# nkwangyh/CubemapSLAM

Measured on AMD Instinct MI355X. Metric: frames/sec (extract+match+localBA) on Lafida cam0, higher is better.
Workload: dtype u8 (extract/match), f64 (BA)

## Files before the change

cubemapslam_amd/api.py:

```python
import time
import ctypes as C
import os
import numpy as np

_HERE = os.path.dirname(os.path.abspath(__file__))
LIB_PATH = os.environ.get("CMS_HIP_LIB") or os.path.join(_HERE, "lib", "libcubemapslam_hip.so")


class CmsError(RuntimeError):
    pass


class Camera(C.Structure):
    _fields_ = [("c", C.c_double), ("d", C.c_double), ("e", C.c_double), ("u0", C.c_double), ("v0", C.c_double),
                ("invpol", C.c_double * 12), ("pol", C.c_double * 5), ("Iw", C.c_int), ("Ih", C.c_int),
                ("face", C.c_int), ("fov_deg", C.c_double)]


class OrbParams(C.Structure):
    _fields_ = [("nfeatures", C.c_int), ("scale_factor", C.c_float), ("nlevels", C.c_int),
                ("ini_th_fast", C.c_int), ("min_th_fast", C.c_int)]


class Geometry(C.Structure):
# ... 795 lines not shown
        return lib().cms_ba_stream(self.h)

    def set_stream(self, hip_stream):
        f = lib().cms_ba_set_stream
        f.argtypes = [C.c_void_p, C.c_void_p]
        _chk(f(self.h, C.c_void_p(int(hip_stream))), "cms_ba_set_stream")

    def profile_kernel(self, kernel_id):
        _chk(lib().cms_ba_profile_kernel(self.h, kernel_id), "cms_ba_profile_kernel")

    def profile_get(self):
        ms = C.c_double(0); n = C.c_long(0)
        _chk(lib().cms_ba_profile_get(self.h, C.byref(ms), C.byref(n)), "cms_ba_profile_get")
        return ms.value, n.value

    def close(self):
        if getattr(self, "h", None) and self.h.value:
            lib().cms_ba_destroy(self.h)
            self.h = C.c_void_p()

    def __del__(self):
        try:
            self.close()
        except Exception:
            pass


def ba_compose_chunks(fixed, n_points, e_pose, e_point, lookahead=48):
    fixed = np.ascontiguousarray(fixed, np.uint8); e_pose = np.ascontiguousarray(e_pose, np.int32); e_point = np.ascontiguousarray(e_point, np.int32)
    P, E = int(n_points), len(e_pose)
# ... 89 lines not shown
    pp = (C.c_void_p * n)(*[o[0].ctypes.data for o in outs]); pq = (C.c_void_p * n)(*[o[1].ctypes.data for o in outs]); pf = (C.c_void_p * n)(*[o[2].ctypes.data for o in outs])
    L = lib()
    L.cms_ba_read_many.argtypes = [C.c_void_p, C.c_int, C.c_void_p, C.c_void_p, C.c_void_p]
    _chk(L.cms_ba_read_many(handles, n, pp, pq, pf), "cms_ba_read_many")
    return outs


def ba_pool_trim(device=0):
    n = C.c_size_t(0)
    L = lib()
    L.cms_ba_pool_trim.argtypes = [C.c_int, C.c_void_p]
    _chk(L.cms_ba_pool_trim(int(device), C.byref(n)), "cms_ba_pool_trim")
    return int(n.value)


def ba_set_deterministic(on):
    _chk(lib().cms_ba_set_deterministic(int(on) if not isinstance(on, bool) else (1 if on else 0)), "cms_ba_set_deterministic")


def ba_get_deterministic():
    return bool(lib().cms_ba_get_deterministic())


def ba_optimize_many(bas, its=(5, 10), stop=None, stop_array=None):
    n = len(bas)
    handles = (C.c_void_p * n)(*[b.h for b in bas])
    stats = (BaStats * n)()
    stop_arr = stop_array if stop_array is not None else (np.array([1], np.uint8) if stop else None)
    lib().cms_ba_optimize_many.argtypes = [C.c_void_p, C.c_int, C.c_int, C.c_int, C.c_void_p, C.c_void_p]
    rc = _chk(lib().cms_ba_optimize_many(handles, n, its[0], its[1], _p(stop_arr), stats), "cms_ba_optimize_many")
# ... 205 lines not shown
```

cubemapslam_amd/csrc/cms_api_ba.hip:

```cpp
#include <algorithm>
#include <cfloat>
#include <chrono>
#include <condition_variable>
#include <deque>
#include <functional>
#include <atomic>
#include <cmath>
#include <mutex>
#include <numeric>
#include <string>
#include <thread>
#include <pthread.h>
#include <unordered_map>
#include "cms_ba_pool.h"

struct BaKnobs {
  bool deterministic, det_points, host_lm, single_host_lm, schur_chunks, schur_points, all_lists, want_all_lists;
  bool no_fused, solve1, trial_points, fixed_ranges, no_permute, create_timing, compose_timing, runs, runs_as_edges, separate_reduce, separate_reduce2, separate_first_pass, rm_valu;
  int solve_reduce_max, leftover_lookahead;
  bool global_sum;
  int lookahead, compose_segments, dup, run_min_chunks, rm_weight, se_waves_cap, em_cost_a, em_cost_b, te_chunks, run_min_pct; bool unified;
  char stream_priority;
  bool run_wg; int rw_waves_cu0, rw_waves_cu1;
};
static const BaKnobs& ba_knobs() {
  static const BaKnobs k = [] {
    BaKnobs q;
    auto on = [](const char* n) { return getenv(n) != nullptr; };
    auto num = [](const char* n, int dflt) { const char* v = getenv(n); return v ? atoi(v) : dflt; };
    q.deterministic = on("CMS_BA_DETERMINISTIC"); q.host_lm = on("CMS_BA_HOST_LM"); q.single_host_lm = on("CMS_BA_SINGLE_HOST_LM");
    q.schur_chunks = on("CMS_BA_SCHUR_CHUNKS"); q.schur_points = on("CMS_BA_SCHUR_POINTS"); q.all_lists = on("CMS_BA_ALL_LISTS");
    q.det_points = on("CMS_BA_DET_POINTS");
    q.want_all_lists = (q.deterministic && q.det_points) || q.host_lm || q.single_host_lm || q.schur_chunks || q.schur_points || q.all_lists;
    q.no_fused = on("CMS_BA_NO_FUSED_LIN"); q.solve1 = on("CMS_BA_SOLVE1"); q.trial_points = on("CMS_BA_TRIAL_POINTS");
    q.fixed_ranges = on("CMS_BA_FIXED_RANGES"); q.no_permute = on("CMS_BA_NO_PERMUTE");
    q.create_timing = on("CMS_BA_CREATE_TIMING"); q.compose_timing = on("CMS_BA_COMPOSE_TIMING");
    q.runs = !on("CMS_BA_NO_RUNS");
    q.runs_as_edges = on("CMS_BA_RUNS_AS_EDGES");
// ... 2 lines not shown
    q.separate_reduce2 = on("CMS_BA_SEPARATE_REDUCE2");
    q.separate_reduce = on("CMS_BA_SEPARATE_REDUCE");
    { const char* v = getenv("CMS_BA_SOLVE_REDUCE_MAX"); q.solve_reduce_max = v ? atoi(v) : 24; }
    q.global_sum = !on("CMS_BA_NO_GLOBAL_SUM");
    q.leftover_lookahead = num("CMS_BA_LEFTOVER_LOOKAHEAD", 0);
    q.lookahead = num("CMS_BA_LOOKAHEAD", 24); q.compose_segments = num("CMS_BA_COMPOSE_SEGMENTS", 0); q.dup = num("CMS_BA_DUP", 0);
    q.run_min_chunks = std::max(1, num("CMS_BA_RUN_MIN_CHUNKS", q.rm_valu ? 2 : 1));
    q.run_min_pct = std::max(10, std::min(100, num("CMS_BA_RUN_MIN_PCT", 100)));
    q.rm_weight = std::max(10, std::min(400, num("CMS_BA_RM_WEIGHT", 58)));
    q.unified = !on("CMS_BA_SPLIT_WORKGROUPS");
    q.em_cost_a = num("CMS_BA_EM_COST_A", 40); q.em_cost_b = num("CMS_BA_EM_COST_B", 30);
    q.te_chunks = std::max(1, std::min(16, num("CMS_BA_TE_CHUNKS", 2)));
    q.se_waves_cap = num("CMS_BA_SE_WAVES", 0);
    q.run_wg = on("CMS_BA_RUN_WG");
    q.rw_waves_cu0 = std::max(1, std::min(32, num("CMS_BA_RW_WAVES0", 12))); q.rw_waves_cu1 = std::max(1, std::min(32, num("CMS_BA_RW_WAVES1", 8)));
    const char* pr = getenv("CMS_BA_STREAM_PRIORITY");
    q.stream_priority = pr ? pr[0] : 0;
    return q;
  }();
  return k;
}

struct BaExpand;
struct BaDevPlan;
struct BaCreateOpts {
  hipStream_t setup_stream = nullptr;
  bool inputs_pinned = false;
  bool force_host_plan = false;
  BaDevPlan* dev_plan = nullptr;
  BaExpand* defer_expand = nullptr;
// ... 25 lines not shown
  int* d_sp_pair_slots = nullptr; double* d_sp_partial = nullptr; double* d_sp_sum = nullptr; int* d_sp_chunk_off = nullptr;
  int sp_threads = 0; size_t sp_lds = 0;
  BaSe se = {};
  int* d_se_chunk_e0 = nullptr; uint32_t* d_se_info = nullptr; double* d_se_partial = nullptr; double* d_se_bp_partial = nullptr; double* d_se_sum = nullptr; int* d_se_pob = nullptr; int* d_se_chunk_off = nullptr;
  int* d_se_lone = nullptr; int4* d_rm_chunk = nullptr; uint2* d_run_lane = nullptr; uint32_t* d_run_mf = nullptr; uint32_t* d_run_fl = nullptr; uint32_t* d_rm_cost = nullptr;
  uint32_t* d_run_fg = nullptr; int* d_rm_cut = nullptr;
  size_t se_lds_fixed = 0; int se_waves = 0;
  size_t rm_lds = 0; int n_runs = 0, rm_points = 0;
  char* h_stage = nullptr; size_t h_stage_bytes = 0;
  int cur = 0;
  double* h_pin = nullptr; size_t h_pin_bytes = 0;
  void* grp_items_dev = nullptr; void* grp_items_host = nullptr; double* grp_scal_dev = nullptr; double* grp_scal_host = nullptr;
  void* grp_lm_dev = nullptr; void* grp_lm_host = nullptr;
  int grp_cap = 0;
  int prof_kernel = 0; std::vector<hipEvent_t> prof_ev; double prof_ms = 0; long prof_launches = 0;
  bool fast_plan = false;
  int* d_raw_pose = nullptr; int* d_raw_point = nullptr; int8_t* d_raw_face = nullptr; int* d_prank = nullptr; int* d_cpo = nullptr; int* d_cedge = nullptr;
  uint8_t* d_pcopy = nullptr; uint8_t* d_lo_copy = nullptr; uint64_t* d_run_sig = nullptr; int* d_iperm = nullptr;
  bool dev_plan = false;
  int* d_plan_counts = nullptr; int* h_plan_counts = nullptr; size_t h_plan_counts_bytes = 0;
  long long* d_plan_clk = nullptr;
  bool se_only = false;
  bool deterministic = false;
  int det_ranges = 0;
  bool det_points = false;
  hipEvent_t ev_setup = nullptr;
  bool setup_wait_pending = false;
  hipStream_t grp_stream = nullptr;
  bool async_pending = false;
  bool gsum_clean = false;
// ... 1615 lines not shown
```

cubemapslam_amd/csrc/cms_api_ba_lm.hip:

```cpp

struct BaLm {
  int iterations = 0, robust = 0;
  double delta = 0;
  int it = 0, qmax = 0, nBad = 0, done = 0, next = 0;
  double lambda = -1, ni = 2, currentChi = 0, iniChi = 0, rho = 0;
  double chi_ini = 0, chi_fin = 0, lam_fin = 0;
};

static bool ba_stopped(const volatile uint8_t* stop) { return stop && *stop; }

static int ba_enqueue_iter_start(cms_ba* b, const BaLm& st) {
  hipStream_t s = b->stream;
  const int cur = b->cur;
  ba_errors(b, cur, st.robust, st.delta, 0);
  hipLaunchKernelGGL(k_ba_lin_points, dim3(b->nblk_p), dim3(128), 0, s, b->d, (const double*)b->d_poses[cur],
                     (const double*)b->d_pts[cur], st.robust, st.delta, b->d_Hll, b->d_bl, b->d_Hpl);
  hipLaunchKernelGGL(k_ba_lin_poses, dim3(b->K, BA_POSE_CHUNKS), dim3(256), 0, s, b->d, (const double*)b->d_poses[cur],
                     (const double*)b->d_pts[cur], st.robust, st.delta, b->d_pose_partial);
  if (b->np > 0)
    hipLaunchKernelGGL(k_ba_pose_finish, dim3(b->np), dim3(64), 0, s, b->np, (const double*)b->d_pose_partial, b->d_Hpp, b->d_bp);
  if (st.it == 0) {
    HIPCHK(hipMemsetAsync(b->d_scal + 3, 0, sizeof(double), s));
    hipLaunchKernelGGL(k_ba_maxdiag, dim3(64), dim3(256), 0, s, b->np, b->P, (const double*)b->d_Hpp, (const double*)b->d_Hll, b->d_scal + 3);
  }
// ... 121 lines not shown
  return true;
}
static int ba_group_reserve(cms_ba* owner, int n) {
  if (owner->grp_cap >= n) return CMS_OK;
  if (owner->grp_items_host) ba_pin_give(owner->device, owner->grp_items_host, owner->grp_pin_bytes[0]);
  if (owner->grp_scal_host) ba_pin_give(owner->device, owner->grp_scal_host, owner->grp_pin_bytes[1]);
  if (owner->grp_lm_host) ba_pin_give(owner->device, owner->grp_lm_host, owner->grp_pin_bytes[2]);
  owner->grp_items_host = nullptr; owner->grp_scal_host = nullptr; owner->grp_lm_host = nullptr;
  owner->grp_cap = 0;
  const int cap = std::max(n, 8);
  { char* q = nullptr; int rc = ba_alloc(owner, &q, (size_t)cap * sizeof(BaItem)); if (rc) return rc; owner->grp_items_dev = q; }
  { int rc = ba_alloc(owner, &owner->grp_scal_dev, (size_t)cap * 8); if (rc) return rc; }
  { char* q = nullptr; int rc = ba_alloc(owner, &q, (size_t)cap * sizeof(BaLmDev)); if (rc) return rc; owner->grp_lm_dev = q; }
  HIPCHK(ba_pin_take(owner->device, (size_t)cap * sizeof(BaItem), &owner->grp_items_host, &owner->grp_pin_bytes[0]));
  HIPCHK(ba_pin_take(owner->device, (size_t)cap * 8 * sizeof(double), (void**)&owner->grp_scal_host, &owner->grp_pin_bytes[1]));
  HIPCHK(ba_pin_take(owner->device, (size_t)cap * sizeof(BaLmDev), &owner->grp_lm_host, &owner->grp_pin_bytes[2]));
  n = cap;
  owner->grp_cap = n;
  return CMS_OK;
}
static bool ba_all_sp(cms_ba** bas, int n) {
  for (int w = 0; w < n; ++w) if (bas[w]->sp.R <= 0) return false;
  return true;
}
static bool ba_use_se(cms_ba** bas, int n) {
  if (ba_knobs().host_lm) return false;
  for (int w = 0; w < n; ++w) if (bas[w]->se.nchunks <= 0 || bas[w]->det_points) return false;
  return true;
}
static bool ba_use_te(cms_ba** bas, int n) {
  if (ba_knobs().trial_points || !ba_use_se(bas, n)) return false;
// ... 147 lines not shown
      hipLaunchKernelGGL(kb_ba_trial_solve, dim3(1, 1, n), dim3(384), lds, s, ditems, dyn, (int)BA_PHASE_TRIAL);
      hipLaunchKernelGGL(kb_ba_trial_points, dim3(max_p, 1, n), dim3(128), 0, s, ditems, dyn, (int)BA_PHASE_TRIAL);
      hipLaunchKernelGGL(kb_ba_reduce2, dim3(1, 1, n), dim3(256), 0, s, ditems, dyn, (int)BA_PHASE_TRIAL);
    }
    HIPCHK(hipStreamSynchronize(s));
    for (int w = 0; w < n; ++w) {
      if (dyn.phase[w] == BA_PHASE_IDLE) continue;
      memcpy(bas[w]->h_pin, g->grp_scal_host + 8 * w, 8 * sizeof(double));
      if (dyn.phase[w] == BA_PHASE_ITER) ba_finish_iter_start(bas[w], st[w]);
      else ba_finish_trial(bas[w], st[w], stop);
    }
  }
  HIPCHK(hipGetLastError());
  return CMS_OK;
}
static int ba_optimize_stage_batched_dev(cms_ba** bas, int n, std::vector<BaLm>& st, const volatile uint8_t* stop) {
  cms_ba* g = bas[0];
  hipStream_t s = g->stream;
  const BaItem* ditems = reinterpret_cast<const BaItem*>(g->grp_items_dev);
  int max_e = 0, max_p = 0, max_K = 0, max_np = 0, max_chunks = 0, max_P = 0, max_R = 0, max_spt = 64, max_pairs = 0, max_it = 0;
  size_t lds = 0, sp_lds = 0;
  const bool all_sp = ba_all_sp(bas, n);
  for (int w = 0; w < n; ++w) {
    max_R = std::max(max_R, bas[w]->sp.R); max_spt = std::max(max_spt, bas[w]->sp_threads); max_pairs = std::max(max_pairs, bas[w]->npairs);
    sp_lds = std::max(sp_lds, bas[w]->sp_lds);
    max_e = std::max(max_e, bas[w]->nblk_e); max_p = std::max(max_p, bas[w]->nblk_p); max_K = std::max(max_K, bas[w]->K);
    max_np = std::max(max_np, bas[w]->np); max_chunks = std::max(max_chunks, bas[w]->nchunks); max_P = std::max(max_P, bas[w]->P);
    lds = std::max(lds, bas[w]->blk_lds);
    max_it = std::max(max_it, st[w].iterations);
  }
  BaLmDev* hlm = reinterpret_cast<BaLmDev*>(g->grp_lm_host);
  for (int w = 0; w < n; ++w) {
    BaLmDev& L = hlm[w];
    memset(&L, 0, sizeof(L));
    L.lambda = st[w].lambda; L.ni = st[w].ni; L.it = st[w].it; L.iterations = st[w].iterations; L.nBad = st[w].nBad; L.done = st[w].done;
    L.cur = bas[w]->cur;
    L.next = (st[w].it >= st[w].iterations || ba_stopped(stop)) ? 2 : 0;
  }
  hipLaunchKernelGGL(kb_ba_lm_load, dim3((n + 63) / 64), dim3(64), 0, s, ditems, n, st[0].robust ? 1 : 0);
  BaDyn dyn{};
  memset(&dyn, 0, sizeof(dyn));
  dyn.robust = st[0].robust; dyn.delta = st[0].delta; dyn.chi2_th = 5.991; dyn.set_level = 0; dyn.dev_lm = 1; dyn.fold_finish = 1;
  bool first_round = false;
  for (int w = 0; w < n; ++w) first_round = first_round || st[w].it == 0;
  const BaGroupMode gm = ba_group_mode(bas, n);
  const bool use_se = gm.use_se, use_te = gm.use_te;
  bool iter_phase = true;
  const bool use_s3 = gm.use_s3;
  int s3_threads = 64; size_t lds3 = 0;
  for (int w = 0; w < n; ++w) { s3_threads = std::max(s3_threads, ba_s3_threads(bas[w]->np)); lds3 = std::max(lds3, bas[w]->blk3_lds); }
  {
    static const int solve_kb = [] { const char* v = getenv("CMS_BA_SOLVE_LDS_KB"); return v ? atoi(v) : 0; }();
    if (solve_kb > 0) lds3 = std::max(lds3, std::min((size_t)solve_kb * 1024, (size_t)BA_LDS_CEILING));
  }
// ... 17 lines not shown
  const bool fused = gm.fused;
  const bool solve_reduces = fused && (gm.gsum || (!ba_knobs().separate_reduce && max_seR <= ba_knobs().solve_reduce_max));
  dyn.fused_lin = fused ? 1 : 0;
  {
    static const bool no_presum = getenv("CMS_BA_NO_SOLVE_PRESUM") != nullptr;
    const size_t need = lds3 + (size_t)max_np2 * 42 * sizeof(double);
    if (use_s3 && solve_reduces && !gm.gsum && !no_presum && need <= BA_LDS_CEILING) { dyn.solve_presum = 1; lds3 = need; }
  }
  const bool first_pass = fused && use_te && first_round && !ba_knobs().separate_first_pass;
  dyn.fold_reduce = (use_te && !ba_knobs().separate_reduce2 && ba_knobs().dup == 0) ? 1 : 0;
  int k = 0;
  const int pk = g->prof_kernel;
  const int dup = ba_knobs().dup;
  auto bracket = [&](int id, int which) {
    if (pk != id) return;
    const size_t i = 2 * (size_t)k + which;
    while (g->prof_ev.size() <= i) { hipEvent_t e = nullptr; if (hipEventCreate(&e) != hipSuccess) return; g->prof_ev.push_back(e); }
    hipEventRecord(g->prof_ev[i], s);
  };
  auto enqueue_round = [&]() {
      if (first_round && first_pass) {
        bracket(1, 0);
        hipLaunchKernelGGL(kb_ba_first_pass, dim3(max_Rt, 1, n), dim3(BA_TE_THREADS), te_lds, s, ditems, dyn, (int)BA_PHASE_ITER);
        bracket(1, 1);
        iter_phase = false;
      } else if (first_round) {
        hipLaunchKernelGGL(kb_ba_errors, dim3(max_e, 1, n), dim3(256), 0, s, ditems, dyn, (int)BA_PHASE_ITER);
        hipLaunchKernelGGL(kb_ba_reduce, dim3(1, 1, n), dim3(256), 0, s, ditems, dyn, (int)BA_PHASE_ITER);
      }
      first_round = false;
      if (iter_phase) {
// ... 65 lines not shown
      if (use_te) {
        hipLaunchKernelGGL(kb_ba_trial_edges, dim3(max_Rt, 1, n), dim3(BA_TE_THREADS), te_lds, s, ditems, dyn, (int)BA_PHASE_TRIAL);
        if (dup == 6) hipLaunchKernelGGL(kb_ba_trial_edges, dim3(max_Rt, 1, n), dim3(BA_TE_THREADS), te_lds, s, ditems, dyn, (int)BA_PHASE_TRIAL);
      } else {
        hipLaunchKernelGGL(kb_ba_trial_points, dim3(max_p, 1, n), dim3(128), 0, s, ditems, dyn, (int)BA_PHASE_TRIAL);
        if (dup == 6) hipLaunchKernelGGL(kb_ba_trial_points, dim3(max_p, 1, n), dim3(128), 0, s, ditems, dyn, (int)BA_PHASE_TRIAL);
      }
      bracket(6, 1);
      bracket(7, 0);
      if (!dyn.fold_reduce) hipLaunchKernelGGL(kb_ba_reduce2, dim3(1, 1, n), dim3(256), 0, s, ditems, dyn, (int)BA_PHASE_TRIAL);
      bracket(7, 1);
      ++k;
  };
  const volatile BaLmDev* vh = reinterpret_cast<const volatile BaLmDev*>(hlm);
  hipError_t werr = hipSuccess;
  for (long spins = 0;;) {
    bool any = false;
    for (int w = 0; w < n; ++w) any = any || vh[w].next != 2;
    if (!any || (k > 0 && ba_stopped(stop))) break;
    if (k - vh[0].rounds < (stop ? 1 : 2)) { enqueue_round(); spins = 0; continue; }
    if (spins < 256) std::this_thread::yield();
    else std::this_thread::sleep_for(std::chrono::microseconds(20));
    if ((++spins & 0xFFF) == 0 && hipStreamQuery(s) != hipErrorNotReady) {
      werr = hipStreamSynchronize(s);
      if (werr != hipSuccess || k - vh[0].rounds >= 2) { if (werr == hipSuccess) werr = hipErrorUnknown; break; }
    }
  }
  const hipError_t serr = hipStreamSynchronize(s);
  HIPCHK(werr);
  HIPCHK(serr);
  HIPCHK(hipGetLastError());
  if (pk > 0)
    for (int r = 0; r < k && 2 * (size_t)r + 1 < g->prof_ev.size(); ++r) {
      float ms = 0;
      if (hipEventElapsedTime(&ms, g->prof_ev[2 * r], g->prof_ev[2 * r + 1]) == hipSuccess) { g->prof_ms += ms; ++g->prof_launches; }
    }
  for (int w = 0; w < n; ++w) {
    const BaLmDev& L = hlm[w];
    BaLm& t = st[w];
    t.lambda = L.lambda; t.ni = L.ni; t.currentChi = L.currentChi; t.iniChi = L.iniChi; t.rho = L.rho; t.it = L.it; t.qmax = L.qmax;
    t.nBad = L.nBad; t.done = L.done; t.next = 2;
    if (L.done > 0 || L.it > 0) { t.chi_ini = L.chi_ini; t.chi_fin = L.chi_fin; t.lam_fin = L.lam_fin; }
    if (L.next == 1 && L.qmax > 0 && ba_stopped(stop)) {
      ++t.done; t.chi_ini = L.chi_ini; t.chi_fin = L.currentChi; t.lam_fin = L.lambda;
    }
    bas[w]->cur = L.cur;
  }
  return CMS_OK;
}

static int ba_classify_batched(cms_ba** bas, int n, int set_level, std::vector<int>& counts) {
  cms_ba* g = bas[0];
  hipStream_t s = g->stream;
  BaDyn dyn{};
  memset(&dyn, 0, sizeof(dyn));
  dyn.chi2_th = 5.991; dyn.set_level = set_level;
  int max_e = 0;
  for (int w = 0; w < n; ++w) {
    dyn.phase[w] = BA_PHASE_CLASSIFY; dyn.cur[w] = (uint8_t)bas[w]->cur;
    max_e = std::max(max_e, bas[w]->nblk_e);
  }
  const BaItem* ditems = reinterpret_cast<const BaItem*>(g->grp_items_dev);
  hipLaunchKernelGGL(kb_ba_classify, dim3(max_e, 1, n), dim3(256), 0, s, ditems, dyn, (int)BA_PHASE_CLASSIFY);
  hipLaunchKernelGGL(kb_ba_counts_publish, dim3((n + 63) / 64), dim3(64), 0, s, ditems, n);
  HIPCHK(hipStreamSynchronize(s));
  const BaLmDev* hlm = reinterpret_cast<const BaLmDev*>(g->grp_lm_host);
  counts.resize(n);
  for (int w = 0; w < n; ++w) counts[w] = hlm[w].n_out[set_level ? 0 : 1];
  return CMS_OK;
}

static int ba_optimize_group(cms_ba** bas, int n, int its_robust, int its_final, const volatile uint8_t* stop, cms_ba_stats* stats);
extern "C" int cms_ba_optimize_many(cms_ba** bas, int n, int its_robust, int its_final, const volatile uint8_t* stop, cms_ba_stats* stats) {
  if (!bas || n < 1) return cms_fail(CMS_ERR_ARG, "cms_ba_optimize_many: bad argument");
  for (int w = 0; w < n; ++w) if (!bas[w]) return cms_fail(CMS_ERR_ARG, "null ba");
  auto kind = [&](int w) {
    const cms_ba* b = bas[w];
    int k = b->device * 8 + (b->fast_plan ? 4 : 0) + (b->se.nchunks > 0 ? 2 : 0) + (b->deterministic ? 1 : 0);
    if (b->deterministic) k += 1024 * (1 + (b->det_points ? 1 : 0) + 2 * (b->rm_lds > 0 ? 1 : 0) + 4 * std::max(0, std::min(15, b->se_waves)) + 64 * b->det_ranges);
    return k;
// ... 47 lines not shown
  }
  std::vector<cms_ba_stats> local(n);
  for (int w = 0; w < n; ++w) memset(&local[w], 0, sizeof(cms_ba_stats));
  if (ba_stopped(stop)) {
    if (batched) for (int w = 0; w < n; ++w) bas[w]->gsum_clean = bas[w]->grp_se.gsum != 0;
    if (stats) memcpy(stats, local.data(), n * sizeof(cms_ba_stats));
    return 1;
  }
  const double delta = std::sqrt(5.991);
  std::vector<BaLm> st(n);
  for (int w = 0; w < n; ++w) { st[w] = BaLm(); st[w].iterations = its_robust; st[w].robust = 1; st[w].delta = delta; }
  const bool host_lm = ba_knobs().host_lm;
  for (int w = 0; w < n; ++w)
    if (bas[w]->se_only && (!batched || host_lm || !ba_use_se(bas, n)))
      return cms_fail(CMS_ERR_UNSUPPORTED, "cms_ba_optimize: the window carries only the edge-major work list but another kernel path was selected");
  int rc = batched ? (host_lm ? ba_optimize_stage_batched(bas, n, st, stop) : ba_optimize_stage_batched_dev(bas, n, st, stop)) : ba_optimize_stage_many(bas, n, st, stop);
  if (rc) return rc;
  tick("stage1");
  for (int w = 0; w < n; ++w) {
    local[w].iterations_done[0] = st[w].done; local[w].chi2_initial[0] = st[w].chi_ini; local[w].chi2_final[0] = st[w].chi_fin;
    local[w].lambda_final[0] = st[w].lam_fin;
  }
  std::vector<std::vector<uint8_t>> flags(n);
  std::vector<int> counts(n, 0);
  auto classify = [&](int set_level) -> int {
    if (batched) return ba_classify_batched(bas, n, set_level, counts);
    for (int w = 0; w < n; ++w) {
      cms_ba* b = bas[w];
      HIPCHK(hipSetDevice(b->device));
      flags[w].resize(b->E);
      hipLaunchKernelGGL(k_ba_classify, dim3(b->nblk_e), dim3(256), 0, b->stream, b->d, (const double*)b->d_poses[b->cur],
                         (const double*)b->d_pts[b->cur], 5.991, set_level, b->d_flags);
      HIPCHK(hipMemcpyAsync(flags[w].data(), b->d_flags, b->E, hipMemcpyDeviceToHost, b->stream));
    }
    for (int w = 0; w < n; ++w) HIPCHK(hipStreamSynchronize(bas[w]->stream));
    for (int w = 0; w < n; ++w) { counts[w] = 0; for (int e = 0; e < bas[w]->E; ++e) counts[w] += flags[w][e]; }
    return CMS_OK;
  };
  if (!ba_stopped(stop)) {
    rc = classify(1);
    if (rc) return rc;
    for (int w = 0; w < n; ++w) local[w].n_outliers_mid = counts[w];
    tick("classified");
    for (int w = 0; w < n; ++w) { st[w] = BaLm(); st[w].iterations = its_final; st[w].robust = 0; st[w].delta = delta; }
    rc = batched ? (host_lm ? ba_optimize_stage_batched(bas, n, st, stop) : ba_optimize_stage_batched_dev(bas, n, st, stop)) : ba_optimize_stage_many(bas, n, st, stop);
    if (rc) return rc;
    for (int w = 0; w < n; ++w) {
      local[w].iterations_done[1] = st[w].done; local[w].chi2_initial[1] = st[w].chi_ini; local[w].chi2_final[1] = st[w].chi_fin;
      local[w].lambda_final[1] = st[w].lam_fin;
    }
    tick("stage2");
  }
  rc = classify(0);
  if (rc) return rc;
  tick("classified");
  if (call_timing) fprintf(stderr, "[cms_ba_optimize_many] %d windows:%s\n", n, t_log.c_str());
  for (int w = 0; w < n; ++w) local[w].n_outliers_final = counts[w];
  if (stats) memcpy(stats, local.data(), n * sizeof(cms_ba_stats));
  if (batched)
    for (int w = 0; w < n; ++w) { bas[w]->async_pending = false; bas[w]->grp_stream = nullptr; bas[w]->gsum_clean = bas[w]->grp_se.gsum != 0; }
  return CMS_OK;
// ... 7 lines not shown
```

cubemapslam_amd/csrc/cms_ba_wrappers.hip:

```cpp
#include <hip/hip_runtime.h>
#include <stdint.h>

#define BA_MAX_GROUP 64
struct BaLmDev {
  double lambda, ni, currentChi, iniChi, rho, chi_ini, chi_fin, lam_fin;
  int it, iterations, qmax, nBad, done, next, cur, rounds;
  int n_out[2], pad[2];
};
struct BaItem {
  BaDev d;
  double* poses[2]; double* pts[2];
  double* Hll; double* bl; double* Hpl; double* Hpp; double* bp; double* pose_partial; double* Dinv; double* db;
  double* chunk_sum; double* x; double* partial; double* scal;
  double* hscal;
  const int2* chunk_range; const int2* tup; const int* pair_of_block; const int* pair_chunk_off;
  uint8_t* flags;
  int nblk_e, nblk_p, nchunks, block_free;
  BaSp sp;
  BaSe se;
  BaLmDev* lm; BaLmDev* hlm;
};
template <class T> struct BaGP {
  BA_AS1 T* p;
  __device__ __forceinline__ BaGP() {}
// ... 86 lines not shown
#define BA_ITEM(PHASE, NBLK)                                                                              \
  const int z = blockIdx.z;                                                                               \
  const BaItemG it(items[z]);                                                                             \
  int ba_ph = dyn.phase[z], cur = dyn.cur[z];                                                             \
  double ba_lambda = dyn.lambda[z];                                                                       \
  bool ba_first = dyn.first_iter[z] != 0;                                                                 \
  if (dyn.dev_lm && (PHASE) != BA_PHASE_CLASSIFY) {                                                       \
    const int nx = it.lm->next;                                                                           \
    ba_ph = nx == 0 ? BA_PHASE_ITER : nx == 1 ? BA_PHASE_TRIAL : BA_PHASE_IDLE;                           \
    cur = it.lm->cur; ba_lambda = it.lm->lambda; ba_first = it.lm->it == 0;                               \
  }                                                                                                       \
  if (ba_ph != (PHASE) || (int)blockIdx.x >= (NBLK)) return;                                              \
  const int nxt = cur ^ 1;                                                                                \
  (void)nxt; (void)ba_lambda; (void)ba_first;

__device__ __forceinline__ void ba_lm_after_iter(BaLmDev* L, BaLmDev* H, double chi, double maxdiag) {
  L->currentChi = chi; L->iniChi = chi;
  if (L->it == 0) { L->chi_ini = chi; L->lambda = 1e-5 * maxdiag; L->ni = 2; L->nBad = 0; }
  L->rho = 0; L->qmax = 0; L->next = 1;
  *H = *L;
}
__device__ __forceinline__ void ba_lm_after_trial(BaLmDev* L, BaLmDev* H, double tempChi, double den, int ok2, bool fused_lin = false) {
  if (!ok2) tempChi = 1.7976931348623157e308;
  double rho = (L->currentChi - tempChi) / (den + 1e-3);
  L->rho = rho;
  if (rho > 0 && isfinite(tempChi)) {
    double alpha = 1. - pow(2 * rho - 1, 3.0);
    alpha = fmin(alpha, 2. / 3.);
    L->lambda *= fmax(1. / 3., alpha);
    L->ni = 2; L->currentChi = tempChi;
    L->cur ^= 1;
  } else {
    L->lambda *= L->ni; L->ni *= 2;
  }
  ++L->qmax;
  if (rho < 0 && L->qmax < 10) { L->next = 1; *H = *L; return; }
  ++L->done;
  L->chi_fin = L->currentChi; L->lam_fin = L->lambda;
  bool terminate = (L->qmax == 10 || rho == 0);
  if (!terminate) {
    if ((L->iniChi - L->currentChi) * 1e3 < L->iniChi) ++L->nBad; else L->nBad = 0;
    if (L->nBad >= 3) terminate = true;
  }
  ++L->it;
  L->next = (terminate || L->it >= L->iterations) ? 2 : 0;
  if (fused_lin && L->next == 0) {
    L->iniChi = L->currentChi; L->rho = 0; L->qmax = 0; L->next = 1;
  }
  *H = *L;
}

extern "C" __global__ void __launch_bounds__(256) kb_ba_errors(const BaItem* __restrict__ items, BaDyn dyn, int phase) {
  BA_ITEM(phase, it.nblk_e)
  if (dyn.dev_lm && !ba_first) return;
  ba_errors_body(blockIdx.x, it.nblk_e, it.d, it.poses[cur], it.pts[cur], dyn.robust, dyn.delta, it.partial);
}
extern "C" __global__ void __launch_bounds__(256) kb_ba_reduce(const BaItem* __restrict__ items, BaDyn dyn, int phase) {
  BA_ITEM(phase, 1)
  if (dyn.dev_lm && !ba_first) return;
  ba_reduce_body(0, 1, it.partial, it.nblk_e, it.scal, 0);
}
extern "C" __global__ void __launch_bounds__(128) kb_ba_lin_points(const BaItem* __restrict__ items, BaDyn dyn, int phase) {
  BA_ITEM(phase, it.nblk_p)
  ba_lin_points_body(blockIdx.x, it.nblk_p, it.d, it.poses[cur], it.pts[cur], dyn.robust, dyn.delta, it.Hll, it.bl,
// ... 221 lines not shown
    atomicExch(ticket, 0);
    if (dyn.dev_lm) ba_lm_after_iter(it.lm, it.hlm, chi, mx);
  }
}
__device__ __forceinline__ void kb_ba_reduce2_window(const BaItem* __restrict__ items, const BaDyn& dyn, int phase) {
  BA_ITEM(phase, 1)
  ba_reduce2_body(0, 1, it.partial, it.se.Rt > 0 ? it.se.Rt : it.nblk_p, it.scal, it.hscal);
  ba_trial_publish(it, dyn);
}
extern "C" __global__ void __launch_bounds__(256) kb_ba_reduce2(const BaItem* __restrict__ items, BaDyn dyn, int phase) {
  kb_ba_reduce2_window(items, dyn, phase);
  if (dyn.dev_lm && blockIdx.z == 0 && threadIdx.x == 0) ba_round_count(items);
}
extern "C" __global__ void __launch_bounds__(256) kb_ba_classify(const BaItem* __restrict__ items, BaDyn dyn, int phase) {
  BA_ITEM(phase, it.nblk_e)
  ba_classify_body(blockIdx.x, it.nblk_e, it.d, it.poses[cur], it.pts[cur], dyn.chi2_th, dyn.set_level, it.flags);
  const int e = blockIdx.x * blockDim.x + threadIdx.x;
  const int n = __syncthreads_count(e < it.d.E && it.flags[e] != 0);
  if (threadIdx.x == 0 && n > 0) atomicAdd((int*)&it.lm->n_out[dyn.set_level ? 0 : 1], n);
}
extern "C" __global__ void __launch_bounds__(64) kb_ba_lm_load(const BaItem* __restrict__ items, int n, int clear_counts) {
  const int w = blockIdx.x * blockDim.x + threadIdx.x;
  if (w >= n) return;
  BaLmDev L = *items[w].hlm;
  const BaLmDev old = *items[w].lm;
  L.n_out[0] = clear_counts ? 0 : old.n_out[0];
  L.n_out[1] = clear_counts ? 0 : old.n_out[1];
  *items[w].lm = L;
  reinterpret_cast<int*>(items[w].scal + 7)[0] = 0;
  items[w].scal[6] = 0.0;
  for (int i = 0; i < 6 * items[w].d.np; ++i) items[w].Hpp[i] = 0.0;
}
extern "C" __global__ void __launch_bounds__(64) kb_ba_counts_publish(const BaItem* __restrict__ items, int n) {
  const int w = blockIdx.x * blockDim.x + threadIdx.x;
  if (w >= n) return;
  items[w].hlm->n_out[0] = items[w].lm->n_out[0];
  items[w].hlm->n_out[1] = items[w].lm->n_out[1];
}
```

include/cubemapslam_hip.h:

```cpp
#ifndef CUBEMAPSLAM_HIP_H
#define CUBEMAPSLAM_HIP_H
#include <stddef.h>
#include <stdint.h>
#ifdef __cplusplus
extern "C" {
#endif

#define CMS_OK 0
#define CMS_ERR_ARG (-1)
#define CMS_ERR_HIP (-2)
#define CMS_ERR_UNSUPPORTED (-3)
#define CMS_ERR_OVERFLOW (-4)
#define CMS_ERR_NO_DEVICE (-5)

enum { CMS_FACE_UNKNOWN = -1, CMS_FACE_FRONT = 0, CMS_FACE_LEFT = 1, CMS_FACE_RIGHT = 2, CMS_FACE_UPPER = 3, CMS_FACE_LOWER = 4 };

typedef struct {
  double c, d, e, u0, v0;
  double invpol[12];
  double pol[5];
  int Iw, Ih;
  int face;
  double fov_deg;
} cms_camera;
// ... 81 lines not shown
  int flags;
} cms_ba_window;
#define CMS_BA_INPUTS_PINNED 1
#define CMS_BA_PLAN_ON_DEVICE 2
int cms_ba_create_many(cms_ba** out, int n, int device, const cms_ba_window* windows, int threads);
int cms_ba_read_many(cms_ba** bas, int n, double** poses, double** points, uint8_t** outlier_flags);
int cms_ba_reset(cms_ba* ba);
int cms_ba_optimize(cms_ba* ba, int its_robust, int its_final, const volatile uint8_t* stop, cms_ba_stats* stats);
int cms_ba_optimize_many(cms_ba** bas, int n, int its_robust, int its_final, const volatile uint8_t* stop, cms_ba_stats* stats);
int cms_ba_read(cms_ba* ba, double* poses, double* points, uint8_t* outlier_flags);
void* cms_ba_stream(cms_ba* ba);
int cms_ba_set_stream(cms_ba* ba, void* hip_stream);
int cms_ba_debug_clocks(cms_ba* ba, long long* out16);
int cms_ba_profile_kernel(cms_ba* ba, int kernel_id);
int cms_ba_profile_get(cms_ba* ba, double* total_ms, long* launches);
int cms_ba_debug_compose(int K, const uint8_t* fixed, int P, int E, const int* e_pose, const int* e_point, int lookahead,
                         int* pinv, int* chunk_pt0, int* n_chunks, uint8_t* rank);
int cms_ba_debug_plan(int K, const uint8_t* fixed, int P, int E, const int* e_pose, const int* e_point, int* pinv, int* perm, uint32_t* info,
                      int* chunk_pt0, int* rm_chunk, uint32_t* run_lane, int* counts, uint32_t* run_mf, uint32_t* run_fl);
int cms_ba_debug_fetch_plan(cms_ba* ba, int* pinv, int* perm, uint32_t* info, int* pt_off, int* e_pose, int* e_point, int8_t* e_face, int* chunk_e0,
                            int* rm_chunk, uint32_t* rm_cost, uint32_t* run_mf, uint32_t* run_fl, int* counts);
int cms_ba_debug_plan_fast(int K, const uint8_t* fixed, int P, int E, const int* e_pose, const int* e_point, int* pinv, int* perm, uint32_t* info,
                           int* chunk_pt0, int* rm_chunk, int* counts, uint32_t* run_mf, uint32_t* run_fl);
int cms_ba_debug_run_fg(int K, const uint8_t* fixed, int P, int E, const int* e_pose, const int* e_point, int fast, uint32_t* run_fg, int* rm_cut, int* counts);
int cms_ba_debug_match(int which, int n, const int* slots, int np, int* choice_out);
void cms_ba_destroy(cms_ba* ba);
int cms_ba_pool_trim(int device, size_t* released);
int cms_ba_set_deterministic(int on);
int cms_ba_get_deterministic(void);
int cms_ba_run(int device, int K, double* poses, const uint8_t* fixed, int P, double* points, int E, const int* e_pose,
// ... 153 lines not shown
```

Baseline: 24830.

## Chain BA LM stages on device with stamp-based pacing and handover kernel

Result: no change. 24910 (median of 5 runs) (+0.3%).

```diff
diff --git a/cubemapslam_amd/api.py b/cubemapslam_amd/api.py
--- a/cubemapslam_amd/api.py
+++ b/cubemapslam_amd/api.py
@@ -833,6 +833,13 @@
         _chk(lib().cms_ba_profile_get(self.h, C.byref(ms), C.byref(n)), "cms_ba_profile_get")
         return ms.value, n.value
 
+    def debug_rounds(self):
+        out = (C.c_int * 4)()
+        f = lib().cms_ba_debug_rounds
+        f.argtypes = [C.c_void_p, C.c_void_p]
+        _chk(f(self.h, out), "cms_ba_debug_rounds")
+        return [[out[0], out[1]], [out[2], out[3]]]
+
     def close(self):
         if getattr(self, "h", None) and self.h.value:
             lib().cms_ba_destroy(self.h)
@@ -952,6 +959,13 @@
     return int(n.value)
 
 
+def ba_debug_pace(it, iterations, nxt, stamp, k, depth=2):
+    a = [np.ascontiguousarray(v, np.int32) for v in (it, iterations, nxt, stamp)]
+    f = lib().cms_ba_debug_pace
+    f.argtypes = [C.c_int] + [C.c_void_p] * 4 + [C.c_int, C.c_int]
+    return _chk(f(len(a[0]), *[_p(v) for v in a], int(k), int(depth)), "cms_ba_debug_pace")
+
+
 def ba_set_deterministic(on):
     _chk(lib().cms_ba_set_deterministic(int(on) if not isinstance(on, bool) else (1 if on else 0)), "cms_ba_set_deterministic")
 
diff --git a/cubemapslam_amd/csrc/cms_api_ba.hip b/cubemapslam_amd/csrc/cms_api_ba.hip
--- a/cubemapslam_amd/csrc/cms_api_ba.hip
+++ b/cubemapslam_amd/csrc/cms_api_ba.hip
@@ -22,6 +22,7 @@
   int lookahead, compose_segments, dup, run_min_chunks, rm_weight, se_waves_cap, em_cost_a, em_cost_b, te_chunks, run_min_pct; bool unified;
   char stream_priority;
   bool run_wg; int rw_waves_cu0, rw_waves_cu1;
+  bool pace_old, host_stages;
 };
 static const BaKnobs& ba_knobs() {
   static const BaKnobs k = [] {
@@ -54,6 +55,7 @@
     q.se_waves_cap = num("CMS_BA_SE_WAVES", 0);
     q.run_wg = on("CMS_BA_RUN_WG");
     q.rw_waves_cu0 = std::max(1, std::min(32, num("CMS_BA_RW_WAVES0", 12))); q.rw_waves_cu1 = std::max(1, std::min(32, num("CMS_BA_RW_WAVES1", 8)));
+    q.pace_old = on("CMS_BA_PACE_OLD"); q.host_stages = on("CMS_BA_HOST_STAGES");
     const char* pr = getenv("CMS_BA_STREAM_PRIORITY");
     q.stream_priority = pr ? pr[0] : 0;
     return q;
@@ -109,6 +111,7 @@
   void* grp_lm_dev = nullptr; void* grp_lm_host = nullptr;
   int grp_cap = 0;
   int prof_kernel = 0; std::vector<hipEvent_t> prof_ev; double prof_ms = 0; long prof_launches = 0;
+  int dbg_rounds[4] = {0, 0, 0, 0};
   bool fast_plan = false;
   int* d_raw_pose = nullptr; int* d_raw_point = nullptr; int8_t* d_raw_face = nullptr; int* d_prank = nullptr; int* d_cpo = nullptr; int* d_cedge = nullptr;
   uint8_t* d_pcopy = nullptr; uint8_t* d_lo_copy = nullptr; uint64_t* d_run_sig = nullptr; int* d_iperm = nullptr;
diff --git a/cubemapslam_amd/csrc/cms_api_ba_lm.hip b/cubemapslam_amd/csrc/cms_api_ba_lm.hip
--- a/cubemapslam_amd/csrc/cms_api_ba_lm.hip
+++ b/cubemapslam_amd/csrc/cms_api_ba_lm.hip
@@ -159,7 +159,7 @@
   { char* q = nullptr; int rc = ba_alloc(owner, &q, (size_t)cap * sizeof(BaLmDev)); if (rc) return rc; owner->grp_lm_dev = q; }
   HIPCHK(ba_pin_take(owner->device, (size_t)cap * sizeof(BaItem), &owner->grp_items_host, &owner->grp_pin_bytes[0]));
   HIPCHK(ba_pin_take(owner->device, (size_t)cap * 8 * sizeof(double), (void**)&owner->grp_scal_host, &owner->grp_pin_bytes[1]));
-  HIPCHK(ba_pin_take(owner->device, (size_t)cap * sizeof(BaLmDev), &owner->grp_lm_host, &owner->grp_pin_bytes[2]));
+  HIPCHK(ba_pin_take(owner->device, (size_t)2 * cap * sizeof(BaLmDev), &owner->grp_lm_host, &owner->grp_pin_bytes[2]));
   n = cap;
   owner->grp_cap = n;
   return CMS_OK;
@@ -337,7 +337,54 @@
   HIPCHK(hipGetLastError());
   return CMS_OK;
 }
-static int ba_optimize_stage_batched_dev(cms_ba** bas, int n, std::vector<BaLm>& st, const volatile uint8_t* stop) {
+static int ba_pace(int n, const int* it, const int* iterations, const int* next, const int* stamp, int k, int depth) {
+  int min_s = INT_MAX;
+  for (int w = 0; w < n; ++w) if (next[w] != 2) min_s = std::min(min_s, stamp[w]);
+  if (min_s == INT_MAX) return 2;
+  if (k - min_s >= depth) return 1;
+  for (int w = 0; w < n; ++w) {
+    if (next[w] == 2) continue;
+    const int q = k - stamp[w];
+    if (q <= 0 || it[w] + q < iterations[w]) return 0;
+  }
+  return 1;
+}
+extern "C" int cms_ba_debug_pace(int n, const int* it, const int* iterations, const int* next, const int* stamp, int k, int depth) {
+  if (n < 1 || !it || !iterations || !next || !stamp || k < 0 || depth < 1) return cms_fail(CMS_ERR_ARG, "cms_ba_debug_pace: bad argument");
+  return ba_pace(n, it, iterations, next, stamp, k, depth);
+}
+extern "C" int cms_ba_debug_rounds(cms_ba* b, int* out4) {
+  if (!b || !out4) return cms_fail(CMS_ERR_ARG, "cms_ba_debug_rounds: bad argument");
+  memcpy(out4, b->dbg_rounds, sizeof(b->dbg_rounds));
+  return CMS_OK;
+}
+static BaLmDev ba_lm_start(const BaLm& t, int cur, bool stopped, int stage) {
+  BaLmDev L;
+  memset(&L, 0, sizeof(L));
+  L.lambda = t.lambda; L.ni = t.ni; L.it = t.it; L.iterations = t.iterations; L.nBad = t.nBad; L.done = t.done;
+  L.cur = cur;
+  L.next = (t.it >= t.iterations || stopped) ? 2 : 0;
+  L.stamp = stage << 16;
+  return L;
+}
+static void ba_lm_finish(const BaLmDev& L, BaLm& t, const volatile uint8_t* stop) {
+  t.lambda = L.lambda; t.ni = L.ni; t.currentChi = L.currentChi; t.iniChi = L.iniChi; t.rho = L.rho; t.it = L.it; t.qmax = L.qmax;
+  t.nBad = L.nBad; t.done = L.done; t.next = 2;
+  if (L.done > 0 || L.it > 0) { t.chi_ini = L.chi_ini; t.chi_fin = L.chi_fin; t.lam_fin = L.lam_fin; }
+  if (L.next == 1 && L.qmax > 0 && ba_stopped(stop)) {
+    ++t.done; t.chi_ini = L.chi_ini; t.chi_fin = L.currentChi; t.lam_fin = L.lambda;
+  }
+}
+static void ba_prof_collect(cms_ba* g, int rounds) {
+  if (g->prof_kernel <= 0) return;
+  for (int r = 0; r < rounds && 2 * (size_t)r + 1 < g->prof_ev.size(); ++r) {
+    float ms = 0;
+    if (hipEventElapsedTime(&ms, g->prof_ev[2 * r], g->prof_ev[2 * r + 1]) == hipSuccess) { g->prof_ms += ms; ++g->prof_launches; }
+  }
+}
+#define BA_STAMP_MAX_ITS 6000
+struct BaStageCtl { int stage = 1; bool chained = false; int k_base = 0; int rounds = 0; };
+static int ba_optimize_stage_batched_dev(cms_ba** bas, int n, std::vector<BaLm>& st, const volatile uint8_t* stop, BaStageCtl& ctl) {
   cms_ba* g = bas[0];
   hipStream_t s = g->stream;
   const BaItem* ditems = reinterpret_cast<const BaItem*>(g->grp_items_dev);
@@ -353,14 +400,11 @@
     max_it = std::max(max_it, st[w].iterations);
   }
   BaLmDev* hlm = reinterpret_cast<BaLmDev*>(g->grp_lm_host);
-  for (int w = 0; w < n; ++w) {
-    BaLmDev& L = hlm[w];
-    memset(&L, 0, sizeof(L));
-    L.lambda = st[w].lambda; L.ni = st[w].ni; L.it = st[w].it; L.iterations = st[w].iterations; L.nBad = st[w].nBad; L.done = st[w].done;
-    L.cur = bas[w]->cur;
-    L.next = (st[w].it >= st[w].iterations || ba_stopped(stop)) ? 2 : 0;
-  }
-  hipLaunchKernelGGL(kb_ba_lm_load, dim3((n + 63) / 64), dim3(64), 0, s, ditems, n, st[0].robust ? 1 : 0);
+  const bool handed_over = ctl.chained && ctl.stage == 2;
+  if (!handed_over) {
+    for (int w = 0; w < n; ++w) hlm[w] = ba_lm_start(st[w], bas[w]->cur, ba_stopped(stop), ctl.stage);
+    hipLaunchKernelGGL(kb_ba_lm_load, dim3((n + 63) / 64), dim3(64), 0, s, ditems, n, st[0].robust ? 1 : 0);
+  }
   BaDyn dyn{};
   memset(&dyn, 0, sizeof(dyn));
   dyn.robust = st[0].robust; dyn.delta = st[0].delta; dyn.chi2_th = 5.991; dyn.set_level = 0; dyn.dev_lm = 1; dyn.fold_finish = 1;
@@ -408,7 +452,7 @@
   const int dup = ba_knobs().dup;
   auto bracket = [&](int id, int which) {
     if (pk != id) return;
-    const size_t i = 2 * (size_t)k + which;
+    const size_t i = 2 * (size_t)(ctl.k_base + k) + which;
     while (g->prof_ev.size() <= i) { hipEvent_t e = nullptr; if (hipEventCreate(&e) != hipSuccess) return; g->prof_ev.push_back(e); }
     hipEventRecord(g->prof_ev[i], s);
   };
@@ -504,47 +548,71 @@
   };
   const volatile BaLmDev* vh = reinterpret_cast<const volatile BaLmDev*>(hlm);
   hipError_t werr = hipSuccess;
-  for (long spins = 0;;) {
-    bool any = false;
-    for (int w = 0; w < n; ++w) any = any || vh[w].next != 2;
-    if (!any || (k > 0 && ba_stopped(stop))) break;
-    if (k - vh[0].rounds < (stop ? 1 : 2)) { enqueue_round(); spins = 0; continue; }
-    if (spins < 256) std::this_thread::yield();
-    else std::this_thread::sleep_for(std::chrono::microseconds(20));
-    if ((++spins & 0xFFF) == 0 && hipStreamQuery(s) != hipErrorNotReady) {
-      werr = hipStreamSynchronize(s);
-      if (werr != hipSuccess || k - vh[0].rounds >= 2) { if (werr == hipSuccess) werr = hipErrorUnknown; break; }
-    }
+  const bool pace_old = stop != nullptr || ba_knobs().pace_old || max_it > BA_STAMP_MAX_ITS;
+  if (pace_old && !ctl.chained) {
+    for (long spins = 0;;) {
+      bool any = false;
+      for (int w = 0; w < n; ++w) any = any || vh[w].next != 2;
+      if (!any || (k > 0 && ba_stopped(stop))) break;
+      if (k - vh[0].rounds < (stop ? 1 : 2)) { enqueue_round(); spins = 0; continue; }
+      if (spins < 256) std::this_thread::yield();
+      else std::this_thread::sleep_for(std::chrono::microseconds(20));
+      if ((++spins & 0xFFF) == 0 && hipStreamQuery(s) != hipErrorNotReady) {
+        werr = hipStreamSynchronize(s);
+        if (werr != hipSuccess || k - vh[0].rounds >= 2) { if (werr == hipSuccess) werr = hipErrorUnknown; break; }
+      }
+    }
+  } else {
+    int it_[BA_MAX_GROUP], its_[BA_MAX_GROUP], nx_[BA_MAX_GROUP], sp_[BA_MAX_GROUP];
+    auto decide = [&]() -> int {
+      for (int w = 0; w < n; ++w) {
+        const int s1 = vh[w].stamp;
+        if (BA_STAMP_STAGE(s1) != ctl.stage) { it_[w] = st[w].it; its_[w] = st[w].iterations; nx_[w] = st[w].it >= st[w].iterations ? 2 : 0; sp_[w] = 0; continue; }
+        it_[w] = vh[w].it; its_[w] = vh[w].iterations; nx_[w] = vh[w].next;
+        if (vh[w].stamp != s1) return 1;
+        sp_[w] = BA_STAMP_ROUNDS(s1);
+      }
+      if (!pace_old) return ba_pace(n, it_, its_, nx_, sp_, k, 2);
+      bool any = false;
+      for (int w = 0; w < n; ++w) any = any || nx_[w] != 2;
+      return !any ? 2 : (ctl.k_base + k - vh[0].rounds < 2 ? 0 : 1);
+    };
+    for (long spins = 0;;) {
+      const int d = decide();
+      if (d == 2) break;
+      if (d == 0) { enqueue_round(); spins = 0; continue; }
+      if (spins < 256) std::this_thread::yield();
+      else std::this_thread::sleep_for(std::chrono::microseconds(20));
+      if ((++spins & 0xFFF) == 0 && hipStreamQuery(s) != hipErrorNotReady) {
+        werr = hipStreamSynchronize(s);
+        if (werr != hipSuccess || decide() == 1) { if (werr == hipSuccess) werr = hipErrorUnknown; break; }
+      }
+    }
+  }
+  ctl.rounds = k;
+  if (ctl.chained) {
+    HIPCHK(werr);
+    HIPCHK(hipGetLastError());
+    return CMS_OK;
   }
   const hipError_t serr = hipStreamSynchronize(s);
   HIPCHK(werr);
   HIPCHK(serr);
   HIPCHK(hipGetLastError());
-  if (pk > 0)
-    for (int r = 0; r < k && 2 * (size_t)r + 1 < g->prof_ev.size(); ++r) {
-      float ms = 0;
-      if (hipEventElapsedTime(&ms, g->prof_ev[2 * r], g->prof_ev[2 * r + 1]) == hipSuccess) { g->prof_ms += ms; ++g->prof_launches; }
-    }
+  ba_prof_collect(g, k);
   for (int w = 0; w < n; ++w) {
-    const BaLmDev& L = hlm[w];
-    BaLm& t = st[w];
-    t.lambda = L.lambda; t.ni = L.ni; t.currentChi = L.currentChi; t.iniChi = L.iniChi; t.rho = L.rho; t.it = L.it; t.qmax = L.qmax;
-    t.nBad = L.nBad; t.done = L.done; t.next = 2;
-    if (L.done > 0 || L.it > 0) { t.chi_ini = L.chi_ini; t.chi_fin = L.chi_fin; t.lam_fin = L.lam_fin; }
-    if (L.next == 1 && L.qmax > 0 && ba_stopped(stop)) {
-      ++t.done; t.chi_ini = L.chi_ini; t.chi_fin = L.currentChi; t.lam_fin = L.lambda;
-    }
-    bas[w]->cur = L.cur;
+    ba_lm_finish(hlm[w], st[w], stop);
+    bas[w]->cur = hlm[w].cur;
   }
   return CMS_OK;
 }
 
-static int ba_classify_batched(cms_ba** bas, int n, int set_level, std::vector<int>& counts) {
+static int ba_classify_enqueue(cms_ba** bas, int n, int set_level, bool dev_lm) {
   cms_ba* g = bas[0];
   hipStream_t s = g->stream;
   BaDyn dyn{};
   memset(&dyn, 0, sizeof(dyn));
-  dyn.chi2_th = 5.991; dyn.set_level = set_level;
+  dyn.chi2_th = 5.991; dyn.set_level = set_level; dyn.dev_lm = dev_lm ? 1 : 0;
   int max_e = 0;
   for (int w = 0; w < n; ++w) {
     dyn.phase[w] = BA_PHASE_CLASSIFY; dyn.cur[w] = (uint8_t)bas[w]->cur;
@@ -553,7 +621,13 @@
   const BaItem* ditems = reinterpret_cast<const BaItem*>(g->grp_items_dev);
   hipLaunchKernelGGL(kb_ba_classify, dim3(max_e, 1, n), dim3(256), 0, s, ditems, dyn, (int)BA_PHASE_CLASSIFY);
   hipLaunchKernelGGL(kb_ba_counts_publish, dim3((n + 63) / 64), dim3(64), 0, s, ditems, n);
-  HIPCHK(hipStreamSynchronize(s));
+  return CMS_OK;
+}
+static int ba_classify_batched(cms_ba** bas, int n, int set_level, std::vector<int>& counts) {
+  cms_ba* g = bas[0];
+  const int rc = ba_classify_enqueue(bas, n, set_level, false);
+  if (rc) return rc;
+  HIPCHK(hipStreamSynchronize(g->stream));
   const BaLmDev* hlm = reinterpret_cast<const BaLmDev*>(g->grp_lm_host);
   counts.resize(n);
   for (int w = 0; w < n; ++w) counts[w] = hlm[w].n_out[set_level ? 0 : 1];
@@ -631,8 +705,61 @@
   for (int w = 0; w < n; ++w)
     if (bas[w]->se_only && (!batched || host_lm || !ba_use_se(bas, n)))
       return cms_fail(CMS_ERR_UNSUPPORTED, "cms_ba_optimize: the window carries only the edge-major work list but another kernel path was selected");
-  int rc = batched ? (host_lm ? ba_optimize_stage_batched(bas, n, st, stop) : ba_optimize_stage_batched_dev(bas, n, st, stop)) : ba_optimize_stage_many(bas, n, st, stop);
+  for (int w = 0; w < n; ++w) memset(bas[w]->dbg_rounds, 0, sizeof(bas[w]->dbg_rounds));
+  int dbg[4] = {0, 0, 0, 0};
+  BaStageCtl ctl;
+  auto dbg_stage = [&](int stage, const BaLmDev* blocks) {
+    dbg[2 * stage - 2] = ctl.rounds;
+    for (int w = 0; w < n; ++w) dbg[2 * stage - 1] = std::max(dbg[2 * stage - 1], BA_STAMP_STAGE(blocks[w].stamp) == stage ? BA_STAMP_ROUNDS(blocks[w].stamp) : 0);
+    for (int w = 0; w < n; ++w) memcpy(bas[w]->dbg_rounds, dbg, sizeof(dbg));
+  };
+  if (batched && !host_lm && !stop && !ba_knobs().host_stages && std::max(its_robust, its_final) <= BA_STAMP_MAX_ITS) {
+    cms_ba* g = bas[0];
+    const BaItem* ditems = reinterpret_cast<const BaItem*>(g->grp_items_dev);
+    BaLmDev* hlm = reinterpret_cast<BaLmDev*>(g->grp_lm_host);
+    BaLmDev* save = hlm + g->grp_cap;
+    ctl.chained = true; ctl.stage = 1;
+    int rc = ba_optimize_stage_batched_dev(bas, n, st, nullptr, ctl);
+    if (rc) return rc;
+    const int k1 = ctl.rounds;
+    tick("stage1");
+    rc = ba_classify_enqueue(bas, n, 1, true);
+    if (rc) return rc;
+    std::vector<BaLm> st2(n);
+    for (int w = 0; w < n; ++w) { st2[w] = BaLm(); st2[w].iterations = its_final; st2[w].robust = 0; st2[w].delta = delta; }
+    hipLaunchKernelGGL(kb_ba_stage_handover, dim3((n + 63) / 64), dim3(64), 0, g->stream, ditems, n, save, ba_lm_start(st2[0], 0, false, 2));
+    tick("handed-over");
+    ctl.stage = 2; ctl.k_base = k1;
+    rc = ba_optimize_stage_batched_dev(bas, n, st2, nullptr, ctl);
+    if (rc) return rc;
+    tick("stage2");
+    rc = ba_classify_enqueue(bas, n, 0, true);
+    if (rc) return rc;
+    HIPCHK(hipStreamSynchronize(g->stream));
+    HIPCHK(hipGetLastError());
+    tick("classified");
+    if (call_timing) fprintf(stderr, "[cms_ba_optimize_many] %d windows:%s\n", n, t_log.c_str());
+    const int k2 = ctl.rounds;
+    ba_prof_collect(g, k1 + k2);
+    ctl.rounds = k1; dbg_stage(1, save);
+    ctl.rounds = k2; dbg_stage(2, hlm);
+    for (int w = 0; w < n; ++w) {
+      ba_lm_finish(save[w], st[w], nullptr);
+      ba_lm_finish(hlm[w], st2[w], nullptr);
+      local[w].iterations_done[0] = st[w].done; local[w].chi2_initial[0] = st[w].chi_ini; local[w].chi2_final[0] = st[w].chi_fin; local[w].lambda_final[0] = st[w].lam_fin;
+      local[w].iterations_done[1] = st2[w].done; local[w].chi2_initial[1] = st2[w].chi_ini; local[w].chi2_final[1] = st2[w].chi_fin; local[w].lambda_final[1] = st2[w].lam_fin;
+      local[w].n_outliers_mid = hlm[w].n_out[0]; local[w].n_outliers_final = hlm[w].n_out[1];
+      bas[w]->cur = hlm[w].cur;
+    }
+    if (stats) memcpy(stats, local.data(), n * sizeof(cms_ba_stats));
+    for (int w = 0; w < n; ++w) { bas[w]->async_pending = false; bas[w]->grp_stream = nullptr; bas[w]->gsum_clean = bas[w]->grp_se.gsum != 0; }
+    return CMS_OK;
+  }
+  const bool dev_stage = batched && !host_lm;
+  ctl.stage = 1;
+  int rc = batched ? (host_lm ? ba_optimize_stage_batched(bas, n, st, stop) : ba_optimize_stage_batched_dev(bas, n, st, stop, ctl)) : ba_optimize_stage_many(bas, n, st, stop);
   if (rc) return rc;
+  if (dev_stage) dbg_stage(1, reinterpret_cast<const BaLmDev*>(bas[0]->grp_lm_host));
   tick("stage1");
   for (int w = 0; w < n; ++w) {
     local[w].iterations_done[0] = st[w].done; local[w].chi2_initial[0] = st[w].chi_ini; local[w].chi2_final[0] = st[w].chi_fin;
@@ -660,8 +787,10 @@
     for (int w = 0; w < n; ++w) local[w].n_outliers_mid = counts[w];
     tick("classified");
     for (int w = 0; w < n; ++w) { st[w] = BaLm(); st[w].iterations = its_final; st[w].robust = 0; st[w].delta = delta; }
-    rc = batched ? (host_lm ? ba_optimize_stage_batched(bas, n, st, stop) : ba_optimize_stage_batched_dev(bas, n, st, stop)) : ba_optimize_stage_many(bas, n, st, stop);
+    ctl.stage = 2;
+    rc = batched ? (host_lm ? ba_optimize_stage_batched(bas, n, st, stop) : ba_optimize_stage_batched_dev(bas, n, st, stop, ctl)) : ba_optimize_stage_many(bas, n, st, stop);
     if (rc) return rc;
+    if (dev_stage) dbg_stage(2, reinterpret_cast<const BaLmDev*>(bas[0]->grp_lm_host));
     for (int w = 0; w < n; ++w) {
       local[w].iterations_done[1] = st[w].done; local[w].chi2_initial[1] = st[w].chi_ini; local[w].chi2_final[1] = st[w].chi_fin;
       local[w].lambda_final[1] = st[w].lam_fin;
diff --git a/cubemapslam_amd/csrc/cms_ba_wrappers.hip b/cubemapslam_amd/csrc/cms_ba_wrappers.hip
--- a/cubemapslam_amd/csrc/cms_ba_wrappers.hip
+++ b/cubemapslam_amd/csrc/cms_ba_wrappers.hip
@@ -5,8 +5,11 @@
 struct BaLmDev {
   double lambda, ni, currentChi, iniChi, rho, chi_ini, chi_fin, lam_fin;
   int it, iterations, qmax, nBad, done, next, cur, rounds;
-  int n_out[2], pad[2];
-};
+  int n_out[2];
+  int stamp, pad;
+};
+#define BA_STAMP_STAGE(s) ((s) >> 16)
+#define BA_STAMP_ROUNDS(s) ((s) & 0xFFFF)
 struct BaItem {
   BaDev d;
   double* poses[2]; double* pts[2];
@@ -124,6 +127,14 @@
   const int nxt = cur ^ 1;                                                                                \
   (void)nxt; (void)ba_lambda; (void)ba_first;
 
+__device__ __forceinline__ void ba_lm_mirror(BaLmDev* L, BaLmDev* H, bool counted) {
+  *H = *L;
+  if (!counted) return;
+  const int s = L->stamp + 1;
+  L->stamp = s;
+  __atomic_signal_fence(__ATOMIC_SEQ_CST);
+  *reinterpret_cast<volatile int*>(&H->stamp) = s;
+}
 __device__ __forceinline__ void ba_lm_after_iter(BaLmDev* L, BaLmDev* H, double chi, double maxdiag) {
   L->currentChi = chi; L->iniChi = chi;
   if (L->it == 0) { L->chi_ini = chi; L->lambda = 1e-5 * maxdiag; L->ni = 2; L->nBad = 0; }
@@ -144,7 +155,7 @@
     L->lambda *= L->ni; L->ni *= 2;
   }
   ++L->qmax;
-  if (rho < 0 && L->qmax < 10) { L->next = 1; *H = *L; return; }
+  if (rho < 0 && L->qmax < 10) { L->next = 1; ba_lm_mirror(L, H, true); return; }
   ++L->done;
   L->chi_fin = L->currentChi; L->lam_fin = L->lambda;
   bool terminate = (L->qmax == 10 || rho == 0);
@@ -157,7 +168,7 @@
   if (fused_lin && L->next == 0) {
     L->iniChi = L->currentChi; L->rho = 0; L->qmax = 0; L->next = 1;
   }
-  *H = *L;
+  ba_lm_mirror(L, H, true);
 }
 
 extern "C" __global__ void __launch_bounds__(256) kb_ba_errors(const BaItem* __restrict__ items, BaDyn dyn, int phase) {
@@ -409,6 +420,7 @@
 }
 extern "C" __global__ void __launch_bounds__(256) kb_ba_classify(const BaItem* __restrict__ items, BaDyn dyn, int phase) {
   BA_ITEM(phase, it.nblk_e)
+  if (dyn.dev_lm) cur = it.lm->cur;
   ba_classify_body(blockIdx.x, it.nblk_e, it.d, it.poses[cur], it.pts[cur], dyn.chi2_th, dyn.set_level, it.flags);
   const int e = blockIdx.x * blockDim.x + threadIdx.x;
   const int n = __syncthreads_count(e < it.d.E && it.flags[e] != 0);
@@ -426,6 +438,22 @@
   items[w].scal[6] = 0.0;
   for (int i = 0; i < 6 * items[w].d.np; ++i) items[w].Hpp[i] = 0.0;
 }
+extern "C" __global__ void __launch_bounds__(64) kb_ba_stage_handover(const BaItem* __restrict__ items, int n, BaLmDev* __restrict__ save, BaLmDev init) {
+  const int w = blockIdx.x * blockDim.x + threadIdx.x;
+  if (w >= n) return;
+  const BaLmDev old = *items[w].lm;
+  save[w] = old;
+  BaLmDev L = init;
+  L.cur = old.cur; L.rounds = old.rounds; L.n_out[0] = old.n_out[0]; L.n_out[1] = old.n_out[1];
+  *items[w].lm = L;
+  reinterpret_cast<int*>(items[w].scal + 7)[0] = 0;
+  items[w].scal[6] = 0.0;
+  for (int i = 0; i < 6 * items[w].d.np; ++i) items[w].Hpp[i] = 0.0;
+  L.stamp = old.stamp;
+  *items[w].hlm = L;
+  __atomic_signal_fence(__ATOMIC_SEQ_CST);
+  *reinterpret_cast<volatile int*>(&items[w].hlm->stamp) = init.stamp;
+}
 extern "C" __global__ void __launch_bounds__(64) kb_ba_counts_publish(const BaItem* __restrict__ items, int n) {
   const int w = blockIdx.x * blockDim.x + threadIdx.x;
   if (w >= n) return;
diff --git a/include/cubemapslam_hip.h b/include/cubemapslam_hip.h
--- a/include/cubemapslam_hip.h
+++ b/include/cubemapslam_hip.h
@@ -119,6 +119,8 @@
 int cms_ba_debug_clocks(cms_ba* ba, long long* out16);
 int cms_ba_profile_kernel(cms_ba* ba, int kernel_id);
 int cms_ba_profile_get(cms_ba* ba, double* total_ms, long* launches);
+int cms_ba_debug_pace(int n, const int* it, const int* iterations, const int* next, const int* stamp, int k, int depth);
+int cms_ba_debug_rounds(cms_ba* ba, int* out4);
 int cms_ba_debug_compose(int K, const uint8_t* fixed, int P, int E, const int* e_pose, const int* e_point, int lookahead,
                          int* pinv, int* chunk_pt0, int* n_chunks, uint8_t* rank);
 int cms_ba_debug_plan(int K, const uint8_t* fixed, int P, int E, const int* e_pose, const int* e_point, int* pinv, int* perm, uint32_t* info,
```
